# unixpickle/learn-nerf

Measured on AMD Instinct MI355X. Metric: ray-samples/s (NeRF train step: fwd + bwd + Adam, 4096 rays x 192 samples per GPU), higher is better.
Workload: dtype bf16; 1 GPU; vanilla NeRF coarse64+fine128 train step (BASELINE.json configs[1]); rays_per_gpu=4096, coarse_samples=64, fine_samples=128, global_batch_rays=4096, parallelism=dp1, precision=bf16 MFMA, fp32 accumulate/master weights

## Files before the change

learn-nerf_amd/csrc/fused_chain.h:

```cpp
#pragma once
#include <utility>

#include "common.h"
#include "fast_math.h"
#include "nerf_wgrad.h"

namespace lnrf {
using namespace nl;

typedef __bf16 bf16x8 __attribute__((ext_vector_type(8)));
typedef float f32x16 __attribute__((ext_vector_type(16)));
typedef float f32x4 __attribute__((ext_vector_type(4)));
typedef short s16x4 __attribute__((ext_vector_type(4)));


template <class F, int... I>
__device__ __forceinline__ void static_for_impl(F&& f, std::integer_sequence<int, I...>) {
  (f(std::integral_constant<int, I>{}), ...);
}
template <int N, class F>
__device__ __forceinline__ void static_for(F&& f) {
  static_for_impl(f, std::make_integer_sequence<int, N>{});
}

constexpr int kThreads = kWaves * 64;
constexpr int kStageBytes = kStageFrags * kFragBytes;
constexpr int kSlots = 3;
constexpr int kRingBytes = kSlots * kStageBytes;
constexpr int kBiasLdsOff = kRingBytes;
constexpr int kFragAhead = 4;

extern __shared__ __attribute__((aligned(16))) char smem[];

#ifdef LNRF_TIMELINE
struct Timeline {
  unsigned long long* buf = nullptr;
  int n = 0;
  bool on = false;
  __device__ __forceinline__ void stamp() {
    if (on) {
      const unsigned long long t = __builtin_amdgcn_s_memtime();
      if ((threadIdx.x & 63) == 0) buf[(threadIdx.x >> 6) * 1024 + n] = t;
      ++n;
    }
  }
};
#define LNRF_TL_STAMP(ring) (ring).tl.stamp()
#else
#define LNRF_TL_STAMP(ring) ((void)0)
#endif

__device__ __forceinline__ bf16x8 bits_to_frag(uint4 v) { return __builtin_bit_cast(bf16x8, v); }
__device__ __forceinline__ uint4 frag_to_bits(bf16x8 v) { return __builtin_bit_cast(uint4, v); }
__device__ __forceinline__ bf16x8 zero_frag() { return bits_to_frag(make_uint4(0, 0, 0, 0)); }

// ... 256 lines not shown
      const bf16x8 ahi = ring.template next<c>();
      const bf16x8 alo = ring.template next<c + 1>();
      acc = __builtin_amdgcn_mfma_f32_32x32x16_bf16(alo, bhi(k_), acc, 0, 0, 0);
      acc = __builtin_amdgcn_mfma_f32_32x32x16_bf16(ahi, blo(k_), acc, 0, 0, 0);
      acc = __builtin_amdgcn_mfma_f32_32x32x16_bf16(ahi, bhi(k_), acc, 0, 0, 0);
      __builtin_amdgcn_sched_barrier(0);
    });
    epi(o_, acc);
  });
}


__device__ __forceinline__ bf16x8 tr_frag(const char* frag_even, int lane, int parity, int q) {
  const int g = lane >> 4;
  const int i = lane & 15;
  const int frag = g & 1;
  const int hk = g >> 1;
  const int qp = i >> 2, p = i & 3;
  const int slot_par = parity ^ frag;
  const int c0 = 16 * q + 8 * hk;
  const int ca = c0 + qp, cb = c0 + 4 + qp;
  const char* base = frag_even + frag * kFragBytes;
  const int offa = 256 * (ca >> 3) + 128 * (((ca >> 2) & 1) ^ slot_par) + 64 * (p & 1) + 16 * (ca & 3) + 8 * (p >> 1);
  const int offb = 256 * (cb >> 3) + 128 * (((cb >> 2) & 1) ^ slot_par) + 64 * (p & 1) + 16 * (cb & 3) + 8 * (p >> 1);
  const s16x4 lo = __builtin_amdgcn_ds_read_tr16_b64_v4i16((__attribute__((address_space(3))) s16x4*)(base + offa));
  const s16x4 hi = __builtin_amdgcn_ds_read_tr16_b64_v4i16((__attribute__((address_space(3))) s16x4*)(base + offb));
  typedef short s16x8 __attribute__((ext_vector_type(8)));
  s16x8 v;
  v[0] = lo[0]; v[1] = lo[1]; v[2] = lo[2]; v[3] = lo[3];
  v[4] = hi[0]; v[5] = hi[1]; v[6] = hi[2]; v[7] = hi[3];
  return __builtin_bit_cast(bf16x8, v);
}

template <int NXF, int NYF, int SPI, bool PLAIN = false>
struct WgStage {
  static constexpr int kWgSpi = SPI;
  static constexpr int NF = NXF + NYF;
  static constexpr int PER_WAVE = (NF + kWaves - 1) / kWaves;
  static constexpr int STEP_BYTES = NF * kFragBytes;
  static constexpr int ITER_BYTES = kWgSpi * STEP_BYTES;
  const char* x_base;
  const char* y_base;
  int x_slot0, y_slot0, x_slots, y_slots;
  int64_t t0, n_tiles;
  int64_t iter_stride, t_end;
  int wave, lane;
  uint4 rr[kWgSpi][PER_WAVE];

  __device__ __forceinline__ void load(int64_t iter) {
    const int64_t tb = t0 + iter * iter_stride;
    const int64_t tbc = tb < t_end ? tb : t0;
    const int64_t xo = dump_off(x_slot0, tbc, n_tiles, x_slots), yo = dump_off(y_slot0, tbc, n_tiles, y_slots);
    const __amdgpu_buffer_rsrc_t rx = __builtin_amdgcn_make_buffer_rsrc(const_cast<char*>(x_base) + xo, 0, 0x7FFFFFFF, 0x00020000);
    const __amdgpu_buffer_rsrc_t ry = __builtin_amdgcn_make_buffer_rsrc(const_cast<char*>(y_base) + yo, 0, 0x7FFFFFFF, 0x00020000);
#pragma unroll
    for (int u = 0; u < kWgSpi; ++u) {
      const int64_t tl = tb + u;
      const bool ok = tl < t_end;
      const int64_t ta = ok ? tl : tbc;
      const unsigned keep = ok ? 0xFFFFFFFFu : 0u;
#pragma unroll
      for (int q = 0; q < PER_WAVE; ++q) {
        int f = wave + kWaves * q;
        if constexpr (NF % kWaves != 0) f = f < NF ? f : NF - 1;
        const bool isx = f < NXF;
        const int bo = (int)(isx ? dump_off(x_slot0 + f, ta, n_tiles, x_slots) - xo
                                 : dump_off(y_slot0 + f - NXF, ta, n_tiles, y_slots) - yo);
        const u32x4 v = __builtin_amdgcn_raw_buffer_load_b128(isx ? rx : ry, bo + lane * 16, 0, PLAIN ? 0 : 2);
        rr[u][q] = make_uint4(v[0] & keep, v[1] & keep, v[2] & keep, v[3] & keep);
      }
    }
  }
  template <int B>
  __device__ __forceinline__ void write() {
#pragma unroll
    for (int u = 0; u < kWgSpi; ++u) {
#pragma unroll
      for (int q = 0; q < PER_WAVE; ++q) {
        int f = wave + kWaves * q;
        if constexpr (NF % kWaves != 0) f = f < NF ? f : NF - 1;
        *reinterpret_cast<uint4*>(&smem[B * ITER_BYTES + u * STEP_BYTES + f * kFragBytes + lane * 16]) = rr[u][q];
      }
    }
  }
};

template <int NXF, int NYF, int WI, int WO, int SPI, bool PLAIN, class PB>
__device__ __forceinline__ void wgrad_body(const PB& pb, const char* __restrict__ save,
                                           const char* __restrict__ gdump, int64_t n_tiles,
                                           WgLayout lay, float* __restrict__ slabs) {
  constexpr int NI = NXF / 2, NO = NYF / 2;
  constexpr int TI = (NI + WI - 1) / WI, TO = (NO + WO - 1) / WO;
  constexpr bool FULL_I = TI * WI == NI, FULL_O = TO * WO == NO;
  using Stage = WgStage<NXF, NYF, SPI, PLAIN>;
  constexpr int kWgSpi = SPI;
  static_assert(WI * WO == kWaves, "wave grid");
  static_assert(NXF % 2 == 0 && NYF % 2 == 0, "fragment pairs");

  const int split = blockIdx.x - pb.first_block;

  const int tid = threadIdx.x;
  const int lane = tid & 63;
  const int wave = __builtin_amdgcn_readfirstlane(tid >> 6);
  const int wi = wave / WO, wo = wave % WO;

  const int64_t per = (n_tiles + pb.n_blocks - 1) / pb.n_blocks;
  int64_t t0 = (int64_t)split * per;
  const int64_t t1 = t0 + per < n_tiles ? t0 + per : n_tiles;
  const int64_t steps = t1 > t0 ? t1 - t0 : 0;
  int64_t iters = (steps + kWgSpi - 1) / kWgSpi;
  int64_t iter_stride = kWgSpi, t_end = t1;
  if (lay.interleave) {
    t0 = (int64_t)split * kWgSpi;
    iter_stride = (int64_t)pb.n_blocks * kWgSpi;
    t_end = n_tiles;
    iters = t0 < n_tiles ? (n_tiles - t0 + iter_stride - 1) / iter_stride : 0;
  }

  Stage stg;
  stg.x_base = save;
  stg.y_base = gdump;
  stg.x_slot0 = pb.x_slot0;
  stg.y_slot0 = pb.y_slot0;
  stg.x_slots = lay.x_slots;
  stg.y_slots = lay.y_slots;
  stg.t0 = t0;
  stg.n_tiles = n_tiles;
  stg.iter_stride = iter_stride;
  stg.t_end = t_end;
  stg.wave = wave;
  stg.lane = lane;

// ... 12 lines not shown
#pragma unroll
    for (int u = 0; u < kWgSpi; ++u) {
      const char* buf = smem + bufi * Stage::ITER_BYTES + u * Stage::STEP_BYTES;
#pragma unroll
      for (int q = 0; q < 2; ++q) {
        bf16x8 bf[TO];
#pragma unroll
        for (int b = 0; b < TO; ++b) {
          const int ot = wo + WO * b;
          if (FULL_O || ot < NO) {
            bf[b] = tr_frag(buf + (NXF + 2 * ot) * kFragBytes, lane, ypar, q);
            if (wi == 0) {
#pragma unroll
              for (int j = 0; j < 8; ++j) bsum[b] += (float)bf[b][j];
            }
          }
        }
#pragma unroll
        for (int a = 0; a < TI; ++a) {
          const int it = wi + WI * a;
          if (FULL_I || it < NI) {
            const bf16x8 af = tr_frag(buf + 2 * it * kFragBytes, lane, xpar, q);
#pragma unroll
            for (int b = 0; b < TO; ++b) {
              const int ot = wo + WO * b;
              if (FULL_O || ot < NO)
                acc[a][b] = __builtin_amdgcn_mfma_f32_32x32x16_bf16(af, bf[b], acc[a][b], 0, 0, 0);
            }
          }
        }
      }
    }
  };
  std::integral_constant<int, 0> c0;
  std::integral_constant<int, 1> c1;
  if (iters > 0) {
    stg.load(0);
    stg.template write<0>();
    stg.load(1);
  }
  for (int64_t i = 0; i < iters; i += 2) {
    __syncthreads();
    stg.template write<1>();
    stg.load(i + 2);
    compute(c0);
    __syncthreads();
    stg.template write<0>();
    stg.load(i + 3);
    if (i + 1 < iters) compute(c1);
  }

  float* __restrict__ mine = slabs + ((int64_t)blockIdx.x * kWaves + wave) * kSlabWaveFloats;
#pragma unroll
  for (int a = 0; a < TI; ++a)
#pragma unroll
    for (int b = 0; b < TO; ++b) {
      float4* dst = reinterpret_cast<float4*>(mine + (a * TO + b) * kSlabTileFloats) + lane;
#pragma unroll
      for (int v = 0; v < 4; ++v)
        dst[64 * v] = make_float4(acc[a][b][4 * v], acc[a][b][4 * v + 1], acc[a][b][4 * v + 2], acc[a][b][4 * v + 3]);
    }
  if (wi == 0) {
#pragma unroll
    for (int b = 0; b < TO; ++b) mine[kSlabTileFloats * kSlabMaxTiles + b * 64 + lane] = bsum[b];
  }
}

constexpr int kSlabReduceWaves = 4;
template <int NXF, int NYF, int WI, int WO, class EPI, class PB>
__device__ __forceinline__ void wgrad_reduce_tile(const PB& pb, int w, int j, const float* __restrict__ slabs,
                                                  float* __restrict__ grads, float* lds) {
  if (j >= kWgradWaveTiles<NXF, NYF, WI, WO>) return;
  const int lane = threadIdx.x & 63, q = threadIdx.x >> 6;
  const WgradTile tile = wgrad_tile<NXF, NYF, WI, WO>(w, j);
  if (!tile.real) return;
  const int b = tile.b;
  const float* __restrict__ src = slabs + ((int64_t)pb.first_block * kWaves + w) * kSlabWaveFloats;
  const int64_t blk_stride = (int64_t)kWaves * kSlabWaveFloats;
  float acc[16];
#pragma unroll
  for (int r = 0; r < 16; ++r) acc[r] = 0.0f;
  const bool bias = tile.bias && pb.do_bias;
  float bsum = 0.0f;
  constexpr int U = 4;
  for (int s0 = q; s0 < pb.n_blocks; s0 += U * kSlabReduceWaves) {
// ... 55 lines not shown
```

learn-nerf_amd/csrc/layout_host.cpp:

```cpp
#include <stdint.h>

#include "dense_plan.h"
#include "fast_math.h"
#include "nerf_wgrad.h"
#include "ngp_layout.h"

using namespace lnrf;

static WgradList wgrad_list_of(int which, int64_t n_tiles) {
  return which == 0 ? wgrad_list_split(n_tiles) : which == 1 ? wgrad_list_ls_finish(n_tiles)
       : which == 2 ? wgrad_list_ref_trunk(n_tiles) : which == 3 ? wgrad_list_ref_normal(n_tiles)
                                                                 : wgrad_list_ref_dir(n_tiles);
}
template <int NXF, int NYF, int WI, int WO>
static int64_t wgrad_count_owners(const WgradProblem& pb, int32_t* count, int64_t n) {
  int64_t outside = 0;
  int64_t i;
  auto hit = [&](bool owned) {
    if (!owned) return;
    if (i >= 0 && i < n) ++count[i];
    else ++outside;
  };
  for (int w = 0; w < kWaves; ++w)
    for (int j = 0; j < kWgradWaveTiles<NXF, NYF, WI, WO>; ++j) {
// ... 85 lines not shown
                         kRef3FwdOff, kRef3BiasOff, kRef3NrmOff, kRef3DirOff, kRef3DirBiasOff, kRef3Bytes};
  return what >= 0 && what < 17 ? v[what] : -1;
}
int lnrf_host_xemb_feat(int ks, int h, int j) { return xemb_feat(ks, h, j); }
int lnrf_host_save_slot(int what, int arg) {
  return what == 0 ? kSaveXin : what == 1 ? kSaveH + 16 * arg : what == 2 ? kSaveZ : what == 3 ? kSaveDin
       : what == 4 ? kSaveH10 : what == 5 ? kSaveMask : kSaveSlots;
}
int lnrf_host_grad_slot(int what, int arg) {
  return what == 0 ? kGradDy11 : what == 1 ? kGradDy10m : what == 2 ? grad_dy_slot(arg) : kGradSlots;
}
int lnrf_host_dir_slot(int what) {
  const int v[7] = {kDirSaveXin, kDirSaveH, kDirSaveMask, kDirSaveSlots, kDirGradDy10, kDirGradDy9, kDirGradSlots};
  return what >= 0 && what < 7 ? v[what] : -1;
}
int lnrf_host_demb_feat(int ks, int h, int j) { return demb_feat(ks, h, j); }
int lnrf_host_hidden_feat(int ks, int h, int j) { return hidden_feat(ks, h, j); }
int lnrf_host_dump_info(int what) { return what == 0 ? kFragBytes : what == 1 ? kTileCols : kWaves; }
int lnrf_host_mask_bit(int ks, int j) { return 16 * (ks >> 1) + 8 * (ks & 1) + j; }
int lnrf_host_dump_lane_off(int slot, int c, int hh) { return dump_lane_off(slot, c, hh); }
void lnrf_host_sincos_pe(float r, float* s, float* c) { lnrf::sincos_pe(r, s, c); }

int lnrf_host_wgrad_const(int what) {
  const int v[8] = {kWgradMaxBlocks, kSlabMaxTiles, kSlabMaxTO, kParamCount, kDirW9, kDirB9, kDirW10, kDirB10};
  return v[what];
}
int lnrf_host_wgrad_list(int which, int64_t n_tiles, int32_t* out) {
  const WgradList list = wgrad_list_of(which, n_tiles);
  for (int i = 0; i < list.args.n_problems; ++i) {
    const WgradProblem& pb = list.args.p[i];
    int32_t* o = out + 6 * i;
    o[0] = pb.first_block; o[1] = pb.n_blocks; o[4] = pb.do_bias; o[5] = 0;
    switch (pb.shape) {
#define X(name, id, NXF, NYF, WI, WO, SPI) case name: o[2] = WgShape<name>::TI * WgShape<name>::TO; o[3] = WgShape<name>::TO; break;
      LNRF_WGRAD_SHAPES(X, X)
#undef X
      default: return -1;
    }
    switch (pb.shape) {
#define X(name) case name:
      LNRF_WGRAD_LS_SHAPES(X, X) o[5] = 1; break;
#undef X
      default: break;
    }
  }
  return list.args.n_problems;
}
int64_t lnrf_host_ngp_stream_indices(int stream, int enc_dim, int32_t* out) {
  if (stream < 0 || stream > 2 || !ngp_enc_dim_ok(enc_dim)) return -1;
  const NgpOffsets off = ngp_offsets(enc_dim, 0);
  const int ne = ngp_ne(enc_dim);
  const int64_t n = stream == 2 ? kNgpBiasFloats : (int64_t)kNgpStreamFrags * 512;
  for (int64_t e = 0; out && e < n; ++e) {
    const int g = (int)(e >> 9), lane = (int)((e >> 3) & 63), j = (int)(e & 7);
    out[e] = (int32_t)(stream == 0 ? ngp_fwd_stream_index(g, lane, j, off, enc_dim, ne)
                     : stream == 1 ? ngp_bwd_stream_index(g, lane, j, off, enc_dim, ne) : ngp_bias_index((int)e, off));
  }
  return n;
}
int64_t lnrf_host_ngp_pack_offset(int what) {
  const int64_t v[7] = {kNgpPackBiasOff, kNgpPackBytes, kNgpSplitBiasOff, kNgpSplitBytes, kNgpStreamFrags,
                        kNgpSplitMaxFrags / 2, kNgpMaxParts};
  return what >= 0 && what < 7 ? v[what] : -1;
}
int64_t lnrf_host_ngp_wgrad_owners(int enc_dim, int32_t* count, int64_t n) {
  if (!ngp_enc_dim_ok(enc_dim)) return -1;
  const int64_t dense_off = 1001;
  const NgpWgradArgs a = ngp_wgrad_args(ngp_offsets(enc_dim, dense_off), enc_dim);
  return ngp_count_owners<0>(a.p[0], dense_off, count, n) + ngp_count_owners<1>(a.p[1], dense_off, count, n) +
         ngp_count_owners<2>(a.p[2], dense_off, count, n) + ngp_count_owners<3>(a.p[3], dense_off, count, n) +
         ngp_count_owners<4>(a.p[4], dense_off, count, n);
}
int lnrf_host_ngp_parts_plan(int enc_dim, int32_t* out) {
  if (!ngp_enc_dim_ok(enc_dim)) return -1;
  const NgpPartsPlan pl = ngp_parts_plan(ngp_offsets(enc_dim, 1001), 1001);
  for (int i = 0; i < kNgpLayers; ++i) {
    int32_t* o = out + 4 * i;
    o[0] = kNgpWgrad[i].layer; o[1] = pl.lo[i]; o[2] = pl.hi[i]; o[3] = pl.parts[i];
  }
  return ngp_dense_params(enc_dim);
}
void lnrf_host_gemm_plan(int64_t sa_i, int64_t sa_r, int64_t sb_r, int64_t sb_j, int64_t I, int32_t J, int64_t R,
                         uint32_t a_low, uint32_t b_low, int32_t bf16, int32_t mode, int32_t splits, int64_t* out) {
  const GemmPlan p = gemm_plan(sa_i, sa_r, sb_r, sb_j, I, J, R, a_low, b_low, bf16 != 0, mode, splits);
  const int64_t v[15] = {p.launch, p.big, p.bf16, p.a_fast_r, p.b_fast_r, p.b_aligned, p.kc, p.nsplit, p.lda, p.ldb,
                         p.r_per_split, p.gx, p.gy, p.gz, p.splits};
  for (int i = 0; i < 15; ++i) out[i] = v[i];
}
void lnrf_host_gemm_tile(int64_t I, int32_t J, uint32_t block0, int64_t count, int64_t* out) {
  for (int64_t e = 0; e < count; ++e) {
    const GemmTile t = gemm_big_tile(block0 + (uint32_t)e, (I + BI - 1) / BI, (J + BJ - 1) / BJ);
    out[2 * e] = t.it;
    out[2 * e + 1] = t.jt;
  }
}
int64_t lnrf_host_dense_bwd_weight_scratch_bytes(int64_t m, int32_t k, int32_t n) { return dense_wgrad_scratch_bytes(m, k, n); }
int64_t lnrf_host_gemm_det_scratch_bytes(int64_t I, int32_t J, int64_t R) { return gemm_det_scratch_bytes(I, J, R); }
int64_t lnrf_host_wgrad_owners(int which, int64_t n_tiles, int32_t* count, int64_t n) {
  const WgradList list = wgrad_list_of(which, n_tiles);
  int64_t outside = 0;
  for (int i = 0; i < list.args.n_problems; ++i) {
    const WgradProblem& pb = list.args.p[i];
    switch (pb.shape) {
#define X(name, id, NXF, NYF, WI, WO, SPI) case name: outside += wgrad_count_owners<NXF, NYF, WI, WO>(pb, count, n); break;
      LNRF_WGRAD_SHAPES(X, X)
#undef X
    }
  }
  return outside;
}
}
```

learn-nerf_amd/csrc/nerf_bwd_ls.hip:

```cpp
#include "nerf_chain.h"

namespace lnrf {

constexpr int kLsWaves = 4;
constexpr int kLsThreads = kLsWaves * 64;
constexpr int kLsStages = 8;
constexpr int kLsLag = 2;
constexpr int kLsDist = kLsLag + 1;
constexpr int kLsBufs = kLsDist + 1;
constexpr int kLsTileBytes = 32 * kFragBytes;
constexpr int kLsPollOff = kLsBufs * kLsTileBytes;
constexpr int kLsLds = kLsPollOff + 5 * 256;
constexpr unsigned kLsMaxSpins = 1u << 18;
constexpr int kLsSlabWaveFloats = 16 * kSlabTileFloats + 2 * 64;
constexpr int64_t kLsSlabBlockBytes = (int64_t)kLsWaves * kLsSlabWaveFloats * (int64_t)sizeof(float);
constexpr int kLsCounterStride = 32;

struct LsJob {
  const char* packed;
  const char* save;
  char* gdump;
  unsigned* counters;
  float* slabs;
  unsigned* status;
// ... 511 lines not shown
  if (rc) return rc;
  int pipes[2] = {total, 0};
  if (n_models == 2) {
    const double share = (double)mdl[0].m / (double)(mdl[0].m + mdl[1].m);
    pipes[0] = (int)(total * share + 0.5);
    if (pipes[0] < 1) pipes[0] = 1;
    if (pipes[0] > total - 1) pipes[0] = total - 1;
    pipes[1] = total - pipes[0];
  }
  LsArgs a;
  a.n_jobs = n_models;
  a.total_pipelines = total;
  for (int k = 0; k < n_models; ++k) {
    const LsModel& md = mdl[k];
    const LsJob& j = a.job[k] = ls_job(md.packed, md.save, md.scratch, md.m, pipes[k]);
    if (phases & 1) {
      hipLaunchKernelGGL(nerf_bwd_head_kernel, dim3((unsigned)(j.n_tiles / kWaves)), dim3(kThreads), kHeadLds, st, j.packed,
                         j.save, md.density, md.rgb, md.g_density, md.g_rgb, md.m, j.n_tiles, j.gdump, j.counters,
                         (phases & 2) ? (int)(kLsCounterBytes / sizeof(unsigned)) : 0);
      LNRF_LAUNCH_CHECK();
    }
    if ((phases & 3) == 2) {
      hipError_t e = hipMemsetAsync(j.counters, 0, kLsCounterBytes, st);
      if (e != hipSuccess) return hip_fail(e, "hipMemsetAsync(counters)");
    }
  }
  if (n_models == 1) a.job[1] = a.job[0];
  if (phases & 2) {
    hipLaunchKernelGGL(nerf_bwd_ls_kernel, dim3((unsigned)(total * kLsStages)), dim3(kLsThreads), kLsLds, st, a);
    LNRF_LAUNCH_CHECK();
  }
  if (!(phases & 4)) return LNRF_OK;
  LsFoldArgs fold;
  for (int k = 0; k < n_models; ++k) {
    const LsModel& md = mdl[k];
    const LsJob& j = a.job[k];
    const WgradList w = wgrad_list_ls_finish(j.n_tiles);
    float* small_slabs = ls_small_slabs(md.scratch, md.m);
    rc = launch_nerf_wgrad(w, md.save, md.scratch, j.n_tiles, md.grads, st, WgLayout{kSaveTileSlots, kGradTileSlots, 1},
                           small_slabs, false, false);
    if (rc) return rc;
    fold.w[k] = w.args;
    fold.small_slabs[k] = small_slabs;
    fold.ls_slabs[k] = j.slabs;
    fold.grads[k] = md.grads;
    fold.pipelines[k] = pipes[k];
  }
  if (n_models == 1) {
    fold.w[1] = fold.w[0]; fold.small_slabs[1] = fold.small_slabs[0]; fold.ls_slabs[1] = fold.ls_slabs[0];
    fold.grads[1] = fold.grads[0]; fold.pipelines[1] = fold.pipelines[0];
  }
  const int gx = fold.w[0].n_problems * kWaves * kSlabMaxTiles + kLsStages * 64;
  hipLaunchKernelGGL(nerf_ls_fold_kernel, dim3((unsigned)gx, (unsigned)n_models), dim3(64 * kSlabReduceWaves), 0, st, fold);
  LNRF_LAUNCH_CHECK();
  return LNRF_OK;
}

extern "C" int lnrf_nerf_mlp_bwd_ls(const lnrf_nerf_shape* shape, const void* packed, const void* save,
                                    const float* density, const float* rgb, const float* g_density,
                                    const float* g_rgb, int64_t m, void* scratch, float* grads, int32_t phases,
                                    lnrf_stream_t stream) {
  LNRF_REQUIRE_NERF_SHAPE(shape);
  LNRF_CHECK_ARG(packed && save && density && rgb && g_density && g_rgb && scratch && grads, "null pointer");
  LNRF_CHECK_ARG(m >= 0, "bad m");
  if (m == 0) return LNRF_OK;
  LNRF_CHECK_ARG(phases >= 1 && phases <= 7, "phases: bit 0 head, bit 1 pipeline, bit 2 small problems + fold");
  const LsModel md{packed, save, density, rgb, g_density, g_rgb, m, scratch, grads};
  return ls_backward(&md, 1, phases, as_stream(stream));
}

extern "C" int lnrf_nerf_mlp_bwd_ls2(const lnrf_nerf_shape* shape, const void* packed_a, const void* save_a,
                                     const float* density_a, const float* rgb_a, const float* g_density_a,
                                     const float* g_rgb_a, int64_t m_a, void* scratch_a, float* grads_a,
                                     const void* packed_b, const void* save_b, const float* density_b,
                                     const float* rgb_b, const float* g_density_b, const float* g_rgb_b, int64_t m_b,
                                     void* scratch_b, float* grads_b, int32_t phases, lnrf_stream_t stream) {
  LNRF_REQUIRE_NERF_SHAPE(shape);
  LNRF_CHECK_ARG(packed_a && save_a && density_a && rgb_a && g_density_a && g_rgb_a && scratch_a && grads_a, "null pointer");
  LNRF_CHECK_ARG(packed_b && save_b && density_b && rgb_b && g_density_b && g_rgb_b && scratch_b && grads_b, "null pointer");
  LNRF_CHECK_ARG(m_a > 0 && m_b > 0, "both models need evaluations (use lnrf_nerf_mlp_bwd_ls for one)");
// ... 6 lines not shown
```

learn-nerf_amd/csrc/nerf_chain.h:

```cpp
#pragma once
#include "fused_chain.h"

namespace lnrf {

template <class Put>
__device__ __forceinline__ void x_encode(const float (&px)[3], int h, Put put) {
  static_for<4>([&](auto ks_) {
    constexpr int ks = decltype(ks_)::value;
#pragma unroll
    for (int pp = 0; pp < 4; ++pp) {
      const int p = 4 * ks + pp;
      float s = 0.0f, co = 0.0f;
      if (p < kXPairs) {
        const int pg = kXPairs * h + p;
        const int cd = pg / kXFreqs, f = pg - kXFreqs * cd;
        const float v = cd == 0 ? px[0] : (cd == 1 ? px[1] : px[2]);
        sincos_pe(v * (float)(1 << f), &s, &co);
      }
      put(ks_, 2 * pp, s);
      put(ks_, 2 * pp + 1, co);
    }
  });
}

// ... 97 lines not shown
      });
  bf16x8 dlogit = zero_frag();
  dlogit[0] = (__bf16)gy9;
  gd.store(kGradDy10m + 8, frag_to_bits(dlogit));
  gd.store(kGradDy10m + 9, frag_to_bits(zero_frag()));

  chain_layer<bwd_cons_base(1), bwd_nk(1), bwd_no(1)>(
      ring, [&](auto) { return zero_acc(); },
      [&](auto k_) -> bf16x8 {
        constexpr int ks = decltype(k_)::value;
        if constexpr (ks < 8) return a0[ks];
        else return dlogit;
      },
      [&](auto o_, const f32x16& acc) {
        constexpr int o = decltype(o_)::value;
        a1[2 * o] = acc_to_frag<0, false>(acc);
        a1[2 * o + 1] = acc_to_frag<1, false>(acc);
        gd.store(grad_dy_slot(8) + 2 * o, frag_to_bits(a1[2 * o]));
        gd.store(grad_dy_slot(8) + 2 * o + 1, frag_to_bits(a1[2 * o + 1]));
      });

  if constexpr (HEAD_ONLY) return;
  static_assert(bwd_nk(2) == 16 && bwd_no(2) == 8, "hidden_back");
  static_for<8>([&](auto i_) {
    constexpr int TT = 2 + decltype(i_)::value, l = bwd_dense(TT);
    if constexpr (TT % 2 == 0) hidden_back<bwd_cons_base(TT), l>(ring, a1, a0, relu_mask[l - 1], gd);
    else hidden_back<bwd_cons_base(TT), l>(ring, a0, a1, relu_mask[l - 1], gd);
  });
}

int launch_nerf_wgrad(const WgradList& list, const void* xbuf, const void* ybuf, int64_t n_tiles, float* grads,
                      hipStream_t stream, WgLayout lay, float* slabs, bool plain_loads = false,
                      bool fold = true);

int64_t ls_scratch_bytes(int64_t m);
float* ls_small_slabs(void* scratch, int64_t m);
int launch_ls_pipeline(const void* packed, const void* save, void* scratch, int64_t m, float* grads, hipStream_t stream);

}
```

learn-nerf_amd/csrc/nerf_mlp.hip:

```cpp
#include "nerf_chain.h"

namespace lnrf {

constexpr int kFusedLds = kRingBytes + round_up(kBiasFloats * 4, 1024);
#ifdef LNRF_TIMELINE
__device__ unsigned long long* g_timeline_buf = nullptr;
#endif

struct FwdSeq {
  static constexpr int count = kFwdUsed;
  static constexpr int at(int c) { return fwd_seq(c); }
};

constexpr int kFwdStages = kFwdFrags / kStageFrags;

template <bool SAVE, bool FROM_RAYS, bool HMASKS = true>
__global__ __launch_bounds__(kThreads) void nerf_fwd_kernel(
    const char* __restrict__ packed, const float* __restrict__ xin_g, const float* __restrict__ din_g,
    const float* __restrict__ rays, int64_t ray_stride, const float* __restrict__ ts, int T, int64_t M,
    int64_t n_tiles, float* __restrict__ density, float* __restrict__ rgb, char* __restrict__ save) {
  const auto [lane, wave, c, h, tile, m, valid] = tile_ctx<kWaves>(M);

  stage_bias<kThreads>(packed + kPackBiasOff, kBiasFloats);
  float px[3] = {0, 0, 0}, pd[3] = {0, 0, 0};
// ... 236 lines not shown
  chain_layer_split<fwd_cons_base(10), fwd_nk(10), fwd_no(10)>(
      ring, [&](auto) { return bias_acc(fwd_bias_base(10), h); },
      [&](auto k_) -> bf16x8 { return a1h[decltype(k_)::value]; },
      [&](auto k_) -> bf16x8 { return a1l[decltype(k_)::value]; },
      [&](auto, const f32x16& acc) {
        if (h == 0 && valid) {
          rgb[m * 3 + 0] = tanhf(acc[0]);
          rgb[m * 3 + 1] = tanhf(acc[1]);
          rgb[m * 3 + 2] = tanhf(acc[2]);
        }
      });
}

__global__ __launch_bounds__(kThreads) void nerf_bwd_chain_kernel(
    const char* __restrict__ packed, const char* __restrict__ save, const float* __restrict__ density,
    const float* __restrict__ rgb, const float* __restrict__ g_density, const float* __restrict__ g_rgb,
    int64_t M, int64_t n_tiles, char* __restrict__ gdump) {
  const auto [lane, wave, c, h, tile, m, valid] = tile_ctx<kWaves>(M);

  Ring<kBwdStages, BwdSeq> ring;
  ring.stream = packed + kPackBwdOff;
  ring.wave = wave;
  ring.lane = lane;
#ifdef LNRF_TIMELINE
  ring.tl.buf = g_timeline_buf + 16 * 1024;
  ring.tl.n = 0;
  ring.tl.on = g_timeline_buf != nullptr && blockIdx.x == gridDim.x / 2;
  ring.tl.stamp();
#endif
  const DumpAddr gd{gdump, n_tiles, tile, c, h, kGradTileSlots};
  bwd_chain_tile(ring, gd, save, n_tiles, density, rgb, g_density, g_rgb, M, tile, lane);
}

template <bool PLAIN>
__global__ __launch_bounds__(kThreads) void nerf_wgrad_kernel(WgradArgs args, const char* __restrict__ save,
                                                              const char* __restrict__ gdump, int64_t n_tiles,
                                                              WgLayout lay, float* __restrict__ slabs) {
  WgradProblem pb = args.p[0];
#pragma unroll
  for (int i = 1; i < kMaxProblems; ++i)
    if (i < args.n_problems && (int)blockIdx.x >= args.p[i].first_block) pb = args.p[i];
  switch (pb.shape) {
#define X(name, id, NXF, NYF, WI, WO, SPI) \
  case name: wgrad_body<NXF, NYF, WI, WO, SPI, PLAIN>(pb, save, gdump, n_tiles, lay, slabs); break;
    LNRF_WGRAD_SHAPES(X, default: X)
#undef X
  }
}

__global__ __launch_bounds__(64 * kSlabReduceWaves) void nerf_wgrad_reduce_kernel(WgradArgs args,
                                                                                 const float* __restrict__ slabs,
                                                                                 float* __restrict__ grads) {
  __shared__ float lds[(kSlabReduceWaves - 1) * 17 * 64];
  const int prob = blockIdx.x / (kWaves * kSlabMaxTiles), w = blockIdx.x / kSlabMaxTiles % kWaves, j = blockIdx.x % kSlabMaxTiles;
  const WgradProblem pb = args.p[prob];
  switch (pb.shape) {
#define X(name, id, NXF, NYF, WI, WO, SPI) \
  case name: wgrad_reduce_tile<NXF, NYF, WI, WO, NerfWgradEpi>(pb, w, j, slabs, grads, lds); break;
    LNRF_WGRAD_SHAPES(X, default: X)
#undef X
  }
}

__global__ void nerf_pack_kernel(const float* __restrict__ params, char* __restrict__ packed) {
  constexpr int64_t units_f = (int64_t)kFwdFrags * 64, units_b = (int64_t)kBwdFrags * 64;
  constexpr int64_t total = units_f + units_b + kBiasFloats;
  for (int64_t u = (int64_t)blockIdx.x * blockDim.x + threadIdx.x; u < total; u += (int64_t)gridDim.x * blockDim.x) {
    if (u < units_f + units_b) {
      const bool fwd = u < units_f;
      const int64_t uu = fwd ? u : u - units_f;
      const int g = (int)(uu >> 6), lane = (int)(uu & 63);
      bf16x8 out;
#pragma unroll
      for (int j = 0; j < 8; ++j)
        out[j] = (__bf16)param_or_zero(params, fwd ? fwd_stream_index(g, lane, j, false) : bwd_stream_index(g, lane, j, false));
      *reinterpret_cast<bf16x8*>(packed + (fwd ? kPackFwdOff : kPackBwdOff) + uu * 16) = out;
    } else {
      const int i = (int)(u - units_f - units_b);
      reinterpret_cast<float*>(packed + kPackBiasOff)[i] = param_or_zero(params, bias_block_index(i, false));
    }
  }
}

__global__ void nerf_pack_split_kernel(const float* __restrict__ params, char* __restrict__ packed) {
  const int64_t total_w = (int64_t)kFwd3Frags * 512;
  const int64_t total = total_w + kBiasFloats;
  for (int64_t e = (int64_t)blockIdx.x * blockDim.x + threadIdx.x; e < total;
       e += (int64_t)gridDim.x * blockDim.x) {
    if (e < total_w) {
      const int g = (int)(e >> 9), lane = (int)((e >> 3) & 63), j = (int)(e & 7);
// ... 119 lines not shown
  if (from_rays) {
    rc = set_max_dynamic_lds(nerf_fwd_split_kernel<true>, kFusedLds);
    if (rc) return rc;
    hipLaunchKernelGGL((nerf_fwd_split_kernel<true>), grid, block, kFusedLds, st, (const char*)packed_split, x, d,
                       rays, ray_stride, ts, (int)t, m, density, rgb);
  } else {
    rc = set_max_dynamic_lds(nerf_fwd_split_kernel<false>, kFusedLds);
    if (rc) return rc;
    hipLaunchKernelGGL((nerf_fwd_split_kernel<false>), grid, block, kFusedLds, st, (const char*)packed_split, x, d,
                       rays, ray_stride, ts, (int)t, m, density, rgb);
  }
  LNRF_LAUNCH_CHECK();
  return LNRF_OK;
}

extern "C" int lnrf_nerf_mlp_bwd_chain(const lnrf_nerf_shape* shape, const void* packed, const void* save,
                                       const float* density, const float* rgb, const float* g_density,
                                       const float* g_rgb, int64_t m, void* scratch, lnrf_stream_t stream) {
  LNRF_REQUIRE_NERF_SHAPE(shape);
  LNRF_CHECK_ARG(packed && save && density && rgb && g_density && g_rgb && scratch, "null pointer");
  LNRF_CHECK_ARG(m >= 0, "bad m");
  if (m == 0) return LNRF_OK;
  const int64_t n_tiles = padded_tiles(m);
  hipStream_t st = as_stream(stream);
  int rc = set_max_dynamic_lds(nerf_bwd_chain_kernel, kFusedLds);
  if (rc) return rc;
  hipLaunchKernelGGL(nerf_bwd_chain_kernel, dim3((unsigned)((n_tiles + kWaves - 1) / kWaves)), dim3(kThreads),
                     kFusedLds, st, (const char*)packed, (const char*)save, density, rgb, g_density, g_rgb, m,
                     n_tiles, (char*)scratch);
  LNRF_LAUNCH_CHECK();
  return LNRF_OK;
}

int lnrf::launch_nerf_wgrad(const WgradList& list, const void* xbuf, const void* ybuf, int64_t n_tiles, float* grads,
                            hipStream_t stream, WgLayout lay, float* slabs, bool plain, bool fold) {
  LNRF_CHECK_ARG(slabs != nullptr && list.blocks <= kWgradMaxBlocks, "needs slabs, and holds at most kWgradMaxBlocks of them");
  const int lds = 2 * 2 * 36 * kFragBytes;
  const dim3 grid((unsigned)list.blocks), block(kThreads);
  int rc = plain ? set_max_dynamic_lds(nerf_wgrad_kernel<true>, lds) : set_max_dynamic_lds(nerf_wgrad_kernel<false>, lds);
  if (rc) return rc;
  if (plain)
    hipLaunchKernelGGL(nerf_wgrad_kernel<true>, grid, block, lds, stream, list.args, (const char*)xbuf,
                       (const char*)ybuf, n_tiles, lay, slabs);
  else
    hipLaunchKernelGGL(nerf_wgrad_kernel<false>, grid, block, lds, stream, list.args, (const char*)xbuf,
                       (const char*)ybuf, n_tiles, lay, slabs);
  LNRF_LAUNCH_CHECK();
  if (fold) {
    hipLaunchKernelGGL(nerf_wgrad_reduce_kernel, dim3((unsigned)(list.args.n_problems * kWaves * kSlabMaxTiles)),
                       dim3(64 * kSlabReduceWaves), 0, stream, list.args, (const float*)slabs, grads);
    LNRF_LAUNCH_CHECK();
  }
  return LNRF_OK;
}

extern "C" int lnrf_nerf_mlp_bwd_weights(const lnrf_nerf_shape* shape, const void* save, void* scratch,
                                         int64_t m, float* grads, lnrf_stream_t stream) {
  LNRF_REQUIRE_NERF_SHAPE(shape);
  LNRF_CHECK_ARG(save && scratch && grads, "null pointer");
  LNRF_CHECK_ARG(m >= 0, "bad m");
  if (m == 0) return LNRF_OK;
  const int64_t n_tiles = padded_tiles(m);
  float* slabs = reinterpret_cast<float*>(reinterpret_cast<char*>(scratch) + grad_dump_bytes(m));
  constexpr int64_t kPlainFrom = 16384;
  return launch_nerf_wgrad(wgrad_list_split(n_tiles), save, scratch, n_tiles, grads, as_stream(stream),
                           WgLayout{kSaveTileSlots, kGradTileSlots}, slabs, n_tiles >= kPlainFrom);
}

#ifdef LNRF_TIMELINE
extern "C" int lnrf_debug_set_timeline(void* buf) {
  hipError_t e = hipMemcpyToSymbol(HIP_SYMBOL(lnrf::g_timeline_buf), &buf, sizeof(buf));
  return e == hipSuccess ? LNRF_OK : hip_fail(e, "hipMemcpyToSymbol(g_timeline_buf)");
}
#endif
```

learn-nerf_amd/csrc/nerf_wgrad.h:

```cpp
#pragma once
#include "nerf_layout.h"

namespace lnrf {
using namespace nl;

constexpr int kSlabMaxTiles = 9, kSlabMaxTO = 4;
constexpr int kSlabTileFloats = 64 * 16;
constexpr int kSlabWaveFloats = kSlabMaxTiles * kSlabTileFloats + kSlabMaxTO * 64;
constexpr int64_t kSlabBlockBytes = (int64_t)kWaves * kSlabWaveFloats * (int64_t)sizeof(float);
constexpr int kWgradMaxBlocks = 512;
constexpr int64_t kWgradSlabBytes = kWgradMaxBlocks * kSlabBlockBytes;

#define LNRF_WGRAD_SHAPES(X, X_ELSE)                                                                      \
  X(WG_HIDDEN, 0, 16, 16, 4, 2, 2)                                          \
  X(WG_Z_DY10M, 1, 16, 10, 4, 2, 2)                                                        \
  X(WG_XEMB, 2, 4, 16, 2, 4, 3)                                             \
  X(WG_DEMB_DY10M, 3, 2, 10, 1, 8, 5)                                                  \
  X(WG_DIR9, 5, 18, 8, 4, 2, 2)                                                     \
  X(WG_ZD_DY10M, 6, 18, 10, 4, 2, 2)                                             \
  X(WG_XEMB_DY0_DY5, 7, 4, 32, 2, 4, 2)                                          \
  X_ELSE(WG_H128_DY3, 4, 8, 2, 4, 2, 6)
#define LNRF_WGRAD_LS_SHAPES(X, X_ELSE) X(WG_XEMB_DY0_DY5) X(WG_ZD_DY10M) X_ELSE(WG_H128_DY3)

enum WgradShape : int {
#define X(name, id, nxf, nyf, wi, wo, spi) name = id,
  LNRF_WGRAD_SHAPES(X, X)
#undef X
};
template <WgradShape S>
struct WgShape;
#define X(name, id, nxf, nyf, wi, wo, spi)                                              \
  template <>                                                                           \
  struct WgShape<name> {                                                                \
    static constexpr int NXF = nxf, NYF = nyf, WI = wi, WO = wo, SPI = spi;             \
    static constexpr int TI = (nxf / 2 + wi - 1) / wi, TO = (nyf / 2 + wo - 1) / wo;  \
  };
LNRF_WGRAD_SHAPES(X, X)
#undef X

enum { ROW_HIDDEN = 0, ROW_XEMB = 1, ROW_DEMB = 2, ROW_Z_DEMB = 3 };
enum { COL_256 = 0, COL_DY10M = 1, COL_DY11 = 2, COL_EXPLICIT = 3, COL_DY0_DY5 = 4 };
struct WgradProblem {
  WgradShape shape;
  int x_slot0;
  int y_slot0;
  int dense;
  int row_map;
  int row_off;
  int col_map;
  int do_bias;
  int first_block, n_blocks;
  int w_off, b_off, out_dim, n_rows;
};
constexpr int kMaxProblems = 13;
struct WgradArgs {
  WgradProblem p[kMaxProblems];
  int n_problems;
};

struct NerfWgradEpi {
  static NL_HD void cols(const WgradProblem& pb, int ot, int colr, int& out_idx, int& out_dim, int64_t& w_off,
                         int64_t& b_off) {
    int dense_w = pb.dense;
    if (pb.col_map == COL_DY10M) {
      if (ot < 4) { out_idx = 32 * ot + colr; out_dim = 128; dense_w = 10; }
      else if (colr == 0 && pb.row_map != ROW_DEMB) { out_idx = 0; out_dim = 1; dense_w = 9; }
    } else if (pb.col_map == COL_DY0_DY5) {
// ... 143 lines not shown
```

Baseline: 186.4 million ray-samples/s.

## Add configurable load FIFO depth to wgrad staging and merge two-model wgrad launches

Makes the wgrad staging prefetch depth configurable: loads go into a register FIFO of DEPTH sets, and the tail masking moves from load time to LDS write time. Every shape stays at depth 1 by default, so that path should behave much as before apart from the restructured loop. Separately, the LS finish path now sends both models' wgrad jobs through a single kernel launch, ordering the larger model first, instead of one launch per model. This cuts launch overhead and lets the two models' blocks share the GPU, at the cost of extra job-selection logic in each block. It also adds timeline instrumentation and a host query for the staging config.

```diff
diff --git a/learn-nerf_amd/csrc/fused_chain.h b/learn-nerf_amd/csrc/fused_chain.h
--- a/learn-nerf_amd/csrc/fused_chain.h
+++ b/learn-nerf_amd/csrc/fused_chain.h
@@ -21,6 +21,17 @@
 template <int N, class F>
 __device__ __forceinline__ void static_for(F&& f) {
   static_for_impl(f, std::make_integer_sequence<int, N>{});
+}
+
+template <int K, int N, class F>
+__device__ __forceinline__ void static_while_impl(F&& f) {
+  if constexpr (K < N) {
+    if (f(std::integral_constant<int, K>{})) static_while_impl<K + 1, N>(f);
+  }
+}
+template <int N, class F>
+__device__ __forceinline__ void static_while(F&& f) {
+  static_while_impl<0, N>(f);
 }
 
 constexpr int kThreads = kWaves * 64;
@@ -343,7 +354,7 @@
   return __builtin_bit_cast(bf16x8, v);
 }
 
-template <int NXF, int NYF, int SPI, bool PLAIN = false>
+template <int NXF, int NYF, int SPI, bool PLAIN = false, int DEPTH = 1>
 struct WgStage {
   static constexpr int kWgSpi = SPI;
   static constexpr int NF = NXF + NYF;
@@ -356,8 +367,9 @@
   int64_t t0, n_tiles;
   int64_t iter_stride, t_end;
   int wave, lane;
-  uint4 rr[kWgSpi][PER_WAVE];
-
+  u32x4 rr[DEPTH][kWgSpi][PER_WAVE];
+
+  template <int S>
   __device__ __forceinline__ void load(int64_t iter) {
     const int64_t tb = t0 + iter * iter_stride;
     const int64_t tbc = tb < t_end ? tb : t0;
@@ -367,9 +379,7 @@
 #pragma unroll
     for (int u = 0; u < kWgSpi; ++u) {
       const int64_t tl = tb + u;
-      const bool ok = tl < t_end;
-      const int64_t ta = ok ? tl : tbc;
-      const unsigned keep = ok ? 0xFFFFFFFFu : 0u;
+      const int64_t ta = tl < t_end ? tl : tbc;
 #pragma unroll
       for (int q = 0; q < PER_WAVE; ++q) {
         int f = wave + kWaves * q;
@@ -377,38 +387,85 @@
         const bool isx = f < NXF;
         const int bo = (int)(isx ? dump_off(x_slot0 + f, ta, n_tiles, x_slots) - xo
                                  : dump_off(y_slot0 + f - NXF, ta, n_tiles, y_slots) - yo);
-        const u32x4 v = __builtin_amdgcn_raw_buffer_load_b128(isx ? rx : ry, bo + lane * 16, 0, PLAIN ? 0 : 2);
-        rr[u][q] = make_uint4(v[0] & keep, v[1] & keep, v[2] & keep, v[3] & keep);
+        rr[S][u][q] = __builtin_amdgcn_raw_buffer_load_b128(isx ? rx : ry, bo + lane * 16, 0, PLAIN ? 0 : 2);
       }
     }
   }
-  template <int B>
-  __device__ __forceinline__ void write() {
+  template <int B, int S>
+  __device__ __forceinline__ void write(int64_t iter) {
+    const int64_t tb = t0 + iter * iter_stride;
 #pragma unroll
     for (int u = 0; u < kWgSpi; ++u) {
+      const unsigned keep = tb + u < t_end ? 0xFFFFFFFFu : 0u;
 #pragma unroll
       for (int q = 0; q < PER_WAVE; ++q) {
         int f = wave + kWaves * q;
         if constexpr (NF % kWaves != 0) f = f < NF ? f : NF - 1;
-        *reinterpret_cast<uint4*>(&smem[B * ITER_BYTES + u * STEP_BYTES + f * kFragBytes + lane * 16]) = rr[u][q];
+        const u32x4 v = rr[S][u][q];
+        *reinterpret_cast<uint4*>(&smem[B * ITER_BYTES + u * STEP_BYTES + f * kFragBytes + lane * 16]) =
+            make_uint4(v[0] & keep, v[1] & keep, v[2] & keep, v[3] & keep);
       }
     }
   }
 };
 
-template <int NXF, int NYF, int WI, int WO, int SPI, bool PLAIN, class PB>
-__device__ __forceinline__ void wgrad_body(const PB& pb, const char* __restrict__ save,
+constexpr int kWgradLds = 2 * 2 * 36 * kFragBytes;
+#ifdef LNRF_TIMELINE
+constexpr int kWgTlIters = 16, kWgTlStamps = 4 * kWgTlIters;
+constexpr int kWgTlLdsBytes = kWaves * kWgTlStamps * 8;
+static __device__ unsigned long long* g_wg_timeline_buf = nullptr;
+struct WgTimeline {
+  bool wg = false, on = false;
+  int n = 0, shape = 0, depth = 0;
+  __device__ __forceinline__ unsigned long long* lds() const {
+    return reinterpret_cast<unsigned long long*>(smem + kWgradLds) + (threadIdx.x >> 6) * kWgTlStamps;
+  }
+  __device__ __forceinline__ void begin(int shape_id, bool chosen, int fifo_depth) {
+    wg = chosen && g_wg_timeline_buf != nullptr;
+    shape = shape_id & 7;
+    depth = fifo_depth;
+  }
+  __device__ __forceinline__ void window(int64_t it, int64_t iters) {
+    on = wg && it >= iters / 2 && it < iters / 2 + kWgTlIters;
+  }
+  __device__ __forceinline__ void stamp() {
+    __builtin_amdgcn_sched_barrier(0);
+    if (on) {
+      const unsigned long long t = __builtin_amdgcn_s_memtime();
+      if ((threadIdx.x & 63) == 0) lds()[n] = t;
+      ++n;
+    }
+    __builtin_amdgcn_sched_barrier(0);
+  }
+  __device__ __forceinline__ void flush() {
+    if (!wg) return;
+    const int lane = threadIdx.x & 63, wave = threadIdx.x >> 6;
+    unsigned long long* out = g_wg_timeline_buf + (int64_t)(shape * kWaves + wave) * (1 + kWgTlStamps);
+    if (lane == 0) out[0] = (unsigned long long)n | ((unsigned long long)depth << 32);
+    out[1 + lane] = lane < n ? lds()[lane] : 0ull;
+  }
+};
+#define LNRF_WG_TL_WINDOW(tl, it, iters) (tl).window(it, iters)
+#define LNRF_WG_TL_STAMP(tl) (tl).stamp()
+#else
+#define LNRF_WG_TL_WINDOW(tl, it, iters) ((void)0)
+#define LNRF_WG_TL_STAMP(tl) ((void)0)
+#endif
+
+template <int NXF, int NYF, int WI, int WO, int SPI, int DEPTH, bool PLAIN, class PB>
+__device__ __forceinline__ void wgrad_body(const PB& pb, int bid, const char* __restrict__ save,
                                            const char* __restrict__ gdump, int64_t n_tiles,
                                            WgLayout lay, float* __restrict__ slabs) {
   constexpr int NI = NXF / 2, NO = NYF / 2;
   constexpr int TI = (NI + WI - 1) / WI, TO = (NO + WO - 1) / WO;
   constexpr bool FULL_I = TI * WI == NI, FULL_O = TO * WO == NO;
-  using Stage = WgStage<NXF, NYF, SPI, PLAIN>;
+  using Stage = WgStage<NXF, NYF, SPI, PLAIN, DEPTH>;
   constexpr int kWgSpi = SPI;
   static_assert(WI * WO == kWaves, "wave grid");
   static_assert(NXF % 2 == 0 && NYF % 2 == 0, "fragment pairs");
-
-  const int split = blockIdx.x - pb.first_block;
+  static_assert(DEPTH >= 1 && DEPTH <= 4, "FIFO depth");
+
+  const int split = bid - pb.first_block;
 
   const int tid = threadIdx.x;
   const int lane = tid & 63;
@@ -487,25 +544,40 @@
       }
     }
   };
-  std::integral_constant<int, 0> c0;
-  std::integral_constant<int, 1> c1;
+  constexpr int kUnroll = DEPTH % 2 == 0 ? DEPTH : 2 * DEPTH;
+#ifdef LNRF_TIMELINE
+  WgTimeline tl;
+  tl.begin(pb.shape, bid == pb.first_block + pb.n_blocks / 2, DEPTH);
+#endif
   if (iters > 0) {
-    stg.load(0);
-    stg.template write<0>();
-    stg.load(1);
-  }
-  for (int64_t i = 0; i < iters; i += 2) {
+    static_for<DEPTH>([&](auto s_) { stg.template load<decltype(s_)::value>(decltype(s_)::value); });
+    stg.template write<0, 0>(0);
+    stg.template load<0>(DEPTH);
+  }
+  int64_t i = 0;
+  auto step = [&](auto k_) {
+    constexpr int k = decltype(k_)::value, set = (k + 1) % DEPTH;
+    LNRF_WG_TL_WINDOW(tl, i + k, iters);
     __syncthreads();
-    stg.template write<1>();
-    stg.load(i + 2);
-    compute(c0);
-    __syncthreads();
-    stg.template write<0>();
-    stg.load(i + 3);
-    if (i + 1 < iters) compute(c1);
-  }
-
-  float* __restrict__ mine = slabs + ((int64_t)blockIdx.x * kWaves + wave) * kSlabWaveFloats;
+    LNRF_WG_TL_STAMP(tl);
+    stg.template write<(k + 1) & 1, set>(i + k + 1);
+    LNRF_WG_TL_STAMP(tl);
+    stg.template load<set>(i + k + 1 + DEPTH);
+    LNRF_WG_TL_STAMP(tl);
+    compute(std::integral_constant<int, k & 1>{});
+    LNRF_WG_TL_STAMP(tl);
+  };
+  for (; i + kUnroll <= iters; i += kUnroll) static_for<kUnroll>(step);
+  static_while<kUnroll - 1>([&](auto k_) {
+    if (i + decltype(k_)::value >= iters) return false;
+    step(k_);
+    return true;
+  });
+#ifdef LNRF_TIMELINE
+  tl.flush();
+#endif
+
+  float* __restrict__ mine = slabs + ((int64_t)bid * kWaves + wave) * kSlabWaveFloats;
 #pragma unroll
   for (int a = 0; a < TI; ++a)
 #pragma unroll
diff --git a/learn-nerf_amd/csrc/layout_host.cpp b/learn-nerf_amd/csrc/layout_host.cpp
--- a/learn-nerf_amd/csrc/layout_host.cpp
+++ b/learn-nerf_amd/csrc/layout_host.cpp
@@ -141,7 +141,7 @@
     int32_t* o = out + 6 * i;
     o[0] = pb.first_block; o[1] = pb.n_blocks; o[4] = pb.do_bias; o[5] = 0;
     switch (pb.shape) {
-#define X(name, id, NXF, NYF, WI, WO, SPI) case name: o[2] = WgShape<name>::TI * WgShape<name>::TO; o[3] = WgShape<name>::TO; break;
+#define X(name, id, NXF, NYF, WI, WO, SPI, DEPTH) case name: o[2] = WgShape<name>::TI * WgShape<name>::TO; o[3] = WgShape<name>::TO; break;
       LNRF_WGRAD_SHAPES(X, X)
 #undef X
       default: return -1;
@@ -151,6 +151,19 @@
       LNRF_WGRAD_LS_SHAPES(X, X) o[5] = 1; break;
 #undef X
       default: break;
+    }
+  }
+  return list.args.n_problems;
+}
+int lnrf_host_wgrad_staging(int which, int64_t n_tiles, int32_t* out) {
+  const WgradList list = wgrad_list_of(which, n_tiles);
+  for (int i = 0; i < list.args.n_problems; ++i) {
+    int32_t* o = out + 3 * i;
+    switch (list.args.p[i].shape) {
+#define X(name, id, NXF, NYF, WI, WO, SPI, DEPTH) case name: o[0] = id; o[1] = SPI; o[2] = DEPTH; break;
+      LNRF_WGRAD_SHAPES(X, X)
+#undef X
+      default: return -1;
     }
   }
   return list.args.n_problems;
@@ -211,7 +224,7 @@
   for (int i = 0; i < list.args.n_problems; ++i) {
     const WgradProblem& pb = list.args.p[i];
     switch (pb.shape) {
-#define X(name, id, NXF, NYF, WI, WO, SPI) case name: outside += wgrad_count_owners<NXF, NYF, WI, WO>(pb, count, n); break;
+#define X(name, id, NXF, NYF, WI, WO, SPI, DEPTH) case name: outside += wgrad_count_owners<NXF, NYF, WI, WO>(pb, count, n); break;
       LNRF_WGRAD_SHAPES(X, X)
 #undef X
     }
diff --git a/learn-nerf_amd/csrc/nerf_bwd_ls.hip b/learn-nerf_amd/csrc/nerf_bwd_ls.hip
--- a/learn-nerf_amd/csrc/nerf_bwd_ls.hip
+++ b/learn-nerf_amd/csrc/nerf_bwd_ls.hip
@@ -567,20 +567,22 @@
   }
   if (!(phases & 4)) return LNRF_OK;
   LsFoldArgs fold;
+  const int first = n_models == 2 && mdl[1].m > mdl[0].m ? 1 : 0;
+  WgradLaunch small[2];
   for (int k = 0; k < n_models; ++k) {
     const LsModel& md = mdl[k];
     const LsJob& j = a.job[k];
     const WgradList w = wgrad_list_ls_finish(j.n_tiles);
     float* small_slabs = ls_small_slabs(md.scratch, md.m);
-    rc = launch_nerf_wgrad(w, md.save, md.scratch, j.n_tiles, md.grads, st, WgLayout{kSaveTileSlots, kGradTileSlots, 1},
-                           small_slabs, false, false);
-    if (rc) return rc;
+    small[k ^ first] = WgradLaunch{w, md.save, md.scratch, j.n_tiles, md.grads, small_slabs};
     fold.w[k] = w.args;
     fold.small_slabs[k] = small_slabs;
     fold.ls_slabs[k] = j.slabs;
     fold.grads[k] = md.grads;
     fold.pipelines[k] = pipes[k];
   }
+  rc = launch_nerf_wgrad(small, n_models, st, WgLayout{kSaveTileSlots, kGradTileSlots, 1}, false, false);
+  if (rc) return rc;
   if (n_models == 1) {
     fold.w[1] = fold.w[0]; fold.small_slabs[1] = fold.small_slabs[0]; fold.ls_slabs[1] = fold.ls_slabs[0];
     fold.grads[1] = fold.grads[0]; fold.pipelines[1] = fold.pipelines[0];
diff --git a/learn-nerf_amd/csrc/nerf_chain.h b/learn-nerf_amd/csrc/nerf_chain.h
--- a/learn-nerf_amd/csrc/nerf_chain.h
+++ b/learn-nerf_amd/csrc/nerf_chain.h
@@ -153,6 +153,16 @@
 int launch_nerf_wgrad(const WgradList& list, const void* xbuf, const void* ybuf, int64_t n_tiles, float* grads,
                       hipStream_t stream, WgLayout lay, float* slabs, bool plain_loads = false,
                       bool fold = true);
+struct WgradLaunch {
+  WgradList list{0};
+  const void* xbuf;
+  const void* ybuf;
+  int64_t n_tiles;
+  float* grads;
+  float* slabs;
+};
+int launch_nerf_wgrad(const WgradLaunch* launches, int n_jobs, hipStream_t stream, WgLayout lay, bool plain_loads,
+                      bool fold);
 
 int64_t ls_scratch_bytes(int64_t m);
 float* ls_small_slabs(void* scratch, int64_t m);
diff --git a/learn-nerf_amd/csrc/nerf_mlp.hip b/learn-nerf_amd/csrc/nerf_mlp.hip
--- a/learn-nerf_amd/csrc/nerf_mlp.hip
+++ b/learn-nerf_amd/csrc/nerf_mlp.hip
@@ -292,17 +292,30 @@
   bwd_chain_tile(ring, gd, save, n_tiles, density, rgb, g_density, g_rgb, M, tile, lane);
 }
 
+struct WgradJob {
+  WgradArgs args;
+  const char* save;
+  const char* gdump;
+  int64_t n_tiles;
+  float* slabs;
+  int blocks;
+};
+struct WgradJobs {
+  WgradJob job[2];
+  int n_jobs;
+};
 template <bool PLAIN>
-__global__ __launch_bounds__(kThreads) void nerf_wgrad_kernel(WgradArgs args, const char* __restrict__ save,
-                                                              const char* __restrict__ gdump, int64_t n_tiles,
-                                                              WgLayout lay, float* __restrict__ slabs) {
-  WgradProblem pb = args.p[0];
+__global__ __launch_bounds__(kThreads) void nerf_wgrad_kernel(WgradJobs jobs, WgLayout lay) {
+  const int second = jobs.n_jobs > 1 && (int)blockIdx.x >= jobs.job[0].blocks ? 1 : 0;
+  const WgradJob& jb = jobs.job[second];
+  const int bid = (int)blockIdx.x - (second ? jobs.job[0].blocks : 0);
+  WgradProblem pb = jb.args.p[0];
 #pragma unroll
   for (int i = 1; i < kMaxProblems; ++i)
-    if (i < args.n_problems && (int)blockIdx.x >= args.p[i].first_block) pb = args.p[i];
+    if (i < jb.args.n_problems && bid >= jb.args.p[i].first_block) pb = jb.args.p[i];
   switch (pb.shape) {
-#define X(name, id, NXF, NYF, WI, WO, SPI) \
-  case name: wgrad_body<NXF, NYF, WI, WO, SPI, PLAIN>(pb, save, gdump, n_tiles, lay, slabs); break;
+#define X(name, id, NXF, NYF, WI, WO, SPI, DEPTH) \
+  case name: wgrad_body<NXF, NYF, WI, WO, SPI, DEPTH, PLAIN>(pb, bid, jb.save, jb.gdump, jb.n_tiles, lay, jb.slabs); break;
     LNRF_WGRAD_SHAPES(X, default: X)
 #undef X
   }
@@ -315,7 +328,7 @@
   const int prob = blockIdx.x / (kWaves * kSlabMaxTiles), w = blockIdx.x / kSlabMaxTiles % kWaves, j = blockIdx.x % kSlabMaxTiles;
   const WgradProblem pb = args.p[prob];
   switch (pb.shape) {
-#define X(name, id, NXF, NYF, WI, WO, SPI) \
+#define X(name, id, NXF, NYF, WI, WO, SPI, DEPTH) \
   case name: wgrad_reduce_tile<NXF, NYF, WI, WO, NerfWgradEpi>(pb, w, j, slabs, grads, lds); break;
     LNRF_WGRAD_SHAPES(X, default: X)
 #undef X
@@ -501,26 +514,41 @@
   return LNRF_OK;
 }
 
+int lnrf::launch_nerf_wgrad(const WgradLaunch* launches, int n_jobs, hipStream_t stream, WgLayout lay, bool plain,
+                            bool fold) {
+  LNRF_CHECK_ARG(n_jobs == 1 || n_jobs == 2, "one job or two");
+  WgradJobs jobs;
+  jobs.n_jobs = n_jobs;
+  int blocks = 0;
+  for (int k = 0; k < 2; ++k) {
+    const WgradLaunch& l = launches[k < n_jobs ? k : 0];
+    LNRF_CHECK_ARG(l.slabs != nullptr && l.list.blocks <= kWgradMaxBlocks, "needs slabs, and holds at most kWgradMaxBlocks of them");
+    jobs.job[k] = WgradJob{l.list.args, (const char*)l.xbuf, (const char*)l.ybuf, l.n_tiles, l.slabs, l.list.blocks};
+    if (k < n_jobs) blocks += l.list.blocks;
+  }
+#ifdef LNRF_TIMELINE
+  const int lds = kWgradLds + kWgTlLdsBytes;
+#else
+  const int lds = kWgradLds;
+#endif
+  const dim3 grid((unsigned)blocks), block(kThreads);
+  int rc = plain ? set_max_dynamic_lds(nerf_wgrad_kernel<true>, lds) : set_max_dynamic_lds(nerf_wgrad_kernel<false>, lds);
+  if (rc) return rc;
+  if (plain) hipLaunchKernelGGL(nerf_wgrad_kernel<true>, grid, block, lds, stream, jobs, lay);
+  else hipLaunchKernelGGL(nerf_wgrad_kernel<false>, grid, block, lds, stream, jobs, lay);
+  LNRF_LAUNCH_CHECK();
+  for (int k = 0; fold && k < n_jobs; ++k) {
+    const WgradLaunch& l = launches[k];
+    hipLaunchKernelGGL(nerf_wgrad_reduce_kernel, dim3((unsigned)(l.list.args.n_problems * kWaves * kSlabMaxTiles)),
+                       dim3(64 * kSlabReduceWaves), 0, stream, l.list.args, (const float*)l.slabs, l.grads);
+    LNRF_LAUNCH_CHECK();
+  }
+  return LNRF_OK;
+}
 int lnrf::launch_nerf_wgrad(const WgradList& list, const void* xbuf, const void* ybuf, int64_t n_tiles, float* grads,
                             hipStream_t stream, WgLayout lay, float* slabs, bool plain, bool fold) {
-  LNRF_CHECK_ARG(slabs != nullptr && list.blocks <= kWgradMaxBlocks, "needs slabs, and holds at most kWgradMaxBlocks of them");
-  const int lds = 2 * 2 * 36 * kFragBytes;
-  const dim3 grid((unsigned)list.blocks), block(kThreads);
-  int rc = plain ? set_max_dynamic_lds(nerf_wgrad_kernel<true>, lds) : set_max_dynamic_lds(nerf_wgrad_kernel<false>, lds);
-  if (rc) return rc;
-  if (plain)
-    hipLaunchKernelGGL(nerf_wgrad_kernel<true>, grid, block, lds, stream, list.args, (const char*)xbuf,
-                       (const char*)ybuf, n_tiles, lay, slabs);
-  else
-    hipLaunchKernelGGL(nerf_wgrad_kernel<false>, grid, block, lds, stream, list.args, (const char*)xbuf,
-                       (const char*)ybuf, n_tiles, lay, slabs);
-  LNRF_LAUNCH_CHECK();
-  if (fold) {
-    hipLaunchKernelGGL(nerf_wgrad_reduce_kernel, dim3((unsigned)(list.args.n_problems * kWaves * kSlabMaxTiles)),
-                       dim3(64 * kSlabReduceWaves), 0, stream, list.args, (const float*)slabs, grads);
-    LNRF_LAUNCH_CHECK();
-  }
-  return LNRF_OK;
+  const WgradLaunch one{list, xbuf, ybuf, n_tiles, grads, slabs};
+  return launch_nerf_wgrad(&one, 1, stream, lay, plain, fold);
 }
 
 extern "C" int lnrf_nerf_mlp_bwd_weights(const lnrf_nerf_shape* shape, const void* save, void* scratch,
@@ -541,4 +569,8 @@
   hipError_t e = hipMemcpyToSymbol(HIP_SYMBOL(lnrf::g_timeline_buf), &buf, sizeof(buf));
   return e == hipSuccess ? LNRF_OK : hip_fail(e, "hipMemcpyToSymbol(g_timeline_buf)");
 }
+extern "C" int lnrf_debug_set_wgrad_timeline(void* buf) {
+  hipError_t e = hipMemcpyToSymbol(HIP_SYMBOL(lnrf::g_wg_timeline_buf), &buf, sizeof(buf));
+  return e == hipSuccess ? LNRF_OK : hip_fail(e, "hipMemcpyToSymbol(g_wg_timeline_buf)");
+}
 #endif
diff --git a/learn-nerf_amd/csrc/nerf_wgrad.h b/learn-nerf_amd/csrc/nerf_wgrad.h
--- a/learn-nerf_amd/csrc/nerf_wgrad.h
+++ b/learn-nerf_amd/csrc/nerf_wgrad.h
@@ -11,28 +11,28 @@
 constexpr int kWgradMaxBlocks = 512;
 constexpr int64_t kWgradSlabBytes = kWgradMaxBlocks * kSlabBlockBytes;
 
-#define LNRF_WGRAD_SHAPES(X, X_ELSE)                                                                      \
-  X(WG_HIDDEN, 0, 16, 16, 4, 2, 2)                                          \
-  X(WG_Z_DY10M, 1, 16, 10, 4, 2, 2)                                                        \
-  X(WG_XEMB, 2, 4, 16, 2, 4, 3)                                             \
-  X(WG_DEMB_DY10M, 3, 2, 10, 1, 8, 5)                                                  \
-  X(WG_DIR9, 5, 18, 8, 4, 2, 2)                                                     \
-  X(WG_ZD_DY10M, 6, 18, 10, 4, 2, 2)                                             \
-  X(WG_XEMB_DY0_DY5, 7, 4, 32, 2, 4, 2)                                          \
-  X_ELSE(WG_H128_DY3, 4, 8, 2, 4, 2, 6)
+#define LNRF_WGRAD_SHAPES(X, X_ELSE)                                                                         \
+  X(WG_HIDDEN, 0, 16, 16, 4, 2, 2, 1)                                          \
+  X(WG_Z_DY10M, 1, 16, 10, 4, 2, 2, 1)                                                        \
+  X(WG_XEMB, 2, 4, 16, 2, 4, 3, 1)                                             \
+  X(WG_DEMB_DY10M, 3, 2, 10, 1, 8, 5, 1)                                                  \
+  X(WG_DIR9, 5, 18, 8, 4, 2, 2, 1)                                                     \
+  X(WG_ZD_DY10M, 6, 18, 10, 4, 2, 2, 1)                                           \
+  X(WG_XEMB_DY0_DY5, 7, 4, 32, 2, 4, 2, 1)                                          \
+  X_ELSE(WG_H128_DY3, 4, 8, 2, 4, 2, 6, 1)
 #define LNRF_WGRAD_LS_SHAPES(X, X_ELSE) X(WG_XEMB_DY0_DY5) X(WG_ZD_DY10M) X_ELSE(WG_H128_DY3)
 
 enum WgradShape : int {
-#define X(name, id, nxf, nyf, wi, wo, spi) name = id,
+#define X(name, id, nxf, nyf, wi, wo, spi, depth) name = id,
   LNRF_WGRAD_SHAPES(X, X)
 #undef X
 };
 template <WgradShape S>
 struct WgShape;
-#define X(name, id, nxf, nyf, wi, wo, spi)                                              \
+#define X(name, id, nxf, nyf, wi, wo, spi, depth)                                       \
   template <>                                                                           \
   struct WgShape<name> {                                                                \
-    static constexpr int NXF = nxf, NYF = nyf, WI = wi, WO = wo, SPI = spi;             \
+    static constexpr int NXF = nxf, NYF = nyf, WI = wi, WO = wo, SPI = spi, DEPTH = depth; \
     static constexpr int TI = (nxf / 2 + wi - 1) / wi, TO = (nyf / 2 + wo - 1) / wo;  \
   };
 LNRF_WGRAD_SHAPES(X, X)
```

Result: no change. 186.9 million ray-samples/s, median of 5 (+0.3%).
